# GestaltCogTeam/STEP

Measured on AMD Instinct MI355X. Metric: training windows/sec on PEMS04, horizon-12 MAE parity, 1/2/4/8 MI355X, higher is better.
Workload: dtype f16 (TSFormer Q/K/weights) + bf16 (P, V, GraphWaveNet / graph-learner GEMMs) operands, f32 accumulate

## Files before the change

include/step_hip.h:

```cpp
#ifndef STEP_HIP_H
#define STEP_HIP_H

#include <stdint.h>

#ifdef __cplusplus
extern "C" {
#endif

const char* step_last_error(void);
int step_abi_version(void);

typedef struct StepGemm {
    int M, N, K, batch;
    const void* A; long sam, sak, sab; int a_bf16;
    const void* B; long sbk, sbn, sbb; int b_bf16;
    float* C; long ldc, scn, scb;
    float alpha;
    int accumulate;
    const float* bias; int relu;
    int splitk;
    int a_kblk; long a_kstride;
    int b_kblk; long b_kstride;
    int b_nblk; long b_nstride;
    int c_nblk; long c_nstride;
// ... 42 lines not shown

long step_dgl_global_saved_floats(int N, int T);
long step_dgl_global_work_floats(int N, int T, int backward);
int step_dgl_global_forward(const float* series_nt, int N, int T, const StepDglParams* p, int training,
                            float momentum, float* saved, float* work, float* g, void* stream);
int step_dgl_global_backward(const float* series_nt, int N, int T, const StepDglParams* p, const float* saved,
                             const float* dg, float* work, const StepDglParams* grads, void* stream);
#define STEP_DGL_FRESH_FC_GRAD 16
int step_dgl_global_backward_phase(const float* series_nt, int N, int T, const StepDglParams* p, const float* saved,
                             const float* dg, float* work, const StepDglParams* grads, int phase, void* stream);

typedef struct StepDglShard { int own1; double count1, count2; } StepDglShard;
int step_dgl_global_forward_shard(const float* series_slice, int N, int Ts, const StepDglParams* p, int training, float momentum,
                                  float* saved, float* work, double* sums, float* g, const StepDglShard* shard, int phase,
                                  void* stream);
int step_dgl_global_backward_shard(const float* series_slice, int N, int Ts, const StepDglParams* p, const float* saved,
                                   const float* dg, float* work, const StepDglParams* grads, const StepDglShard* shard, int phase,
                                   void* stream);
long step_dgl_global_offset(int N, int T, int item);

int step_dgl_fc_dgrad(const float* dgpre, const void* wp, const void* a2h, const float* coef, const float* st2, int N, long K,
                      void* dz2h, void* stream);
long step_dgl_fc_dgrad_streams(int N, long K);

long step_dgl_edges_saved_floats(int B, int N);
long step_dgl_edges_work_floats(int N);
long step_dgl_edges_theta_offset(int N);
int step_dgl_edges_forward(const float* g, int N, int B, const StepDglParams* p, const float* u, uint64_t seed,
                           float temperature, float* saved, float* theta_out, float* adj_out, void* stream);
int step_dgl_edges_forward_keyed(const float* g, int N, int B, const StepDglParams* p, const long* key, uint64_t seed,
                                 float temperature, float* saved, float* theta_out, float* adj_out, void* stream);
int step_dgl_edges_backward(const float* g, int N, int B, const StepDglParams* p, const float* saved,
                            const float* dtheta, const float* dadj, float temperature, float* work,
                            const StepDglParams* grads, float* dg, void* aux_stream, void* stream);
int step_dgl_edges_backward_acc(const float* g, int N, int B, const StepDglParams* p, const float* saved,
                                const float* dtheta, const float* dadj, float temperature, float* work,
                                const StepDglParams* grads, float* dg, int dg_accumulate, void* aux_stream, void* stream);

typedef struct StepGwnetParams {
    float *nodevec1, *nodevec2;
    float *start_w, *start_b;
    float *filter_w[8], *filter_b[8];
    float *gate_w[8], *gate_b[8];
    float *skip_w[8], *skip_b[8];
    float *bn_w[8], *bn_b[8], *bn_rm[8], *bn_rv[8];
    float *gconv_w[8], *gconv_b[8];
// ... 171 lines not shown
```

step_amd/_lib.py:

```python
import ctypes
import os

import torch

_HERE = os.path.dirname(os.path.abspath(__file__))
LIB_PATH = os.environ.get("STEP_HIP_LIB") or os.path.join(_HERE, "libstep_hip.so")

_vp, _i, _l, _f, _u64 = ctypes.c_void_p, ctypes.c_int, ctypes.c_long, ctypes.c_float, ctypes.c_uint64


class StepGemm(ctypes.Structure):
    _fields_ = [("M", _i), ("N", _i), ("K", _i), ("batch", _i),
                ("A", _vp), ("sam", _l), ("sak", _l), ("sab", _l), ("a_bf16", _i),
                ("B", _vp), ("sbk", _l), ("sbn", _l), ("sbb", _l), ("b_bf16", _i),
                ("C", _vp), ("ldc", _l), ("scn", _l), ("scb", _l),
                ("alpha", _f), ("accumulate", _i), ("bias", _vp), ("relu", _i), ("splitk", _i),
                ("a_kblk", _i), ("a_kstride", _l), ("b_kblk", _i), ("b_kstride", _l),
                ("b_nblk", _i), ("b_nstride", _l), ("c_nblk", _i), ("c_nstride", _l),
                ("a_kscale", _vp), ("a_kshift", _vp), ("a_kperiod", _i),
                ("batch0", _i), ("sab1", _l), ("sbb1", _l), ("scb1", _l), ("compute_bf16", _i), ("a_rowsum", _vp), ("c_nscale", _vp), ("c_nshift", _vp), ("c_mvec", _vp),
                ("c_nperiod", _i), ("splitk_ws", _vp), ("splitk_ws_floats", _l)]


class StepDglParams(ctypes.Structure):
# ... 31 lines not shown
    "step_last_error": (ctypes.c_char_p, []),
    "step_abi_version": (_i, []),
    "step_gemm": (_i, [ctypes.POINTER(StepGemm), _vp]),
    "step_tsformer_encode": (_i, [_vp, _i, _i, _vp, _l, _i, _i, _vp, _vp, _vp, _vp, _f, _vp, _l, _u64, _vp, _vp]),
    "step_dropout_pool_fill": (_i, [_vp, _l, _f, _u64, _vp]),
    "step_tsformer_dropout_words": (_l, [_i, _i]),
    "step_gather_windows": (_i, [_vp, _i, _i, _i, _i, _vp, _i, _i, _i, _vp, _vp, _vp, _vp]),
    "step_pack_long_history": (_i, [_vp, _i, _i, _i, _i, _i, _vp, _vp]),
    "step_knn_workspace_bytes": (_l, [_i, _i, _i]),
    "step_knn_graph": (_i, [_vp, _vp, _i, _i, _i, _i, _vp, _vp, _vp, _l, _vp]),
    "step_topk_mask": (_i, [_vp, _i, _i, _i, _vp, _vp, _l, _vp]),
    "step_selftest_mfma": (_i, [_vp, _vp]),
    "step_streams_concurrent": (_i, [_vp, _vp, ctypes.POINTER(_i)]),
    "step_dgl_global_saved_floats": (_l, [_i, _i]),
    "step_dgl_global_work_floats": (_l, [_i, _i, _i]),
    "step_dgl_global_forward": (_i, [_vp, _i, _i, _PD, _i, _f, _vp, _vp, _vp, _vp]),
    "step_dgl_global_backward": (_i, [_vp, _i, _i, _PD, _vp, _vp, _vp, _PD, _vp]),
    "step_dgl_global_backward_phase": (_i, [_vp, _i, _i, _PD, _vp, _vp, _vp, _PD, _i, _vp]),
    "step_dgl_global_forward_shard": (_i, [_vp, _i, _i, _PD, _i, _f, _vp, _vp, _vp, _vp, _PS, _i, _vp]),
    "step_dgl_global_backward_shard": (_i, [_vp, _i, _i, _PD, _vp, _vp, _vp, _PD, _PS, _i, _vp]),
    "step_dgl_global_offset": (_l, [_i, _i, _i]),
    "step_dgl_fc_dgrad": (_i, [_vp, _vp, _vp, _vp, _vp, _i, _l, _vp, _vp]),
    "step_dgl_fc_dgrad_streams": (_l, [_i, _l]),
    "step_dgl_edges_saved_floats": (_l, [_i, _i]),
    "step_dgl_edges_work_floats": (_l, [_i]),
    "step_dgl_edges_theta_offset": (_l, [_i]),
    "step_dgl_edges_forward": (_i, [_vp, _i, _i, _PD, _vp, _u64, _f, _vp, _vp, _vp, _vp]),
    "step_dgl_edges_forward_keyed": (_i, [_vp, _i, _i, _PD, _vp, _u64, _f, _vp, _vp, _vp, _vp]),
    "step_dgl_edges_backward": (_i, [_vp, _i, _i, _PD, _vp, _vp, _vp, _f, _vp, _PD, _vp, _vp, _vp]),
    "step_dgl_edges_backward_acc": (_i, [_vp, _i, _i, _PD, _vp, _vp, _vp, _f, _vp, _PD, _vp, _i, _vp, _vp]),
    "step_gwnet_saved_floats": (_l, [_i, _i, _i]),
    "step_gwnet_work_floats": (_l, [_i, _i, _i]),
    "step_gwnet_saved_offset": (_l, [_i, _i, _i, _i, _i]),
    "step_gwnet_forward": (_i, [_vp, _i, _i, _i, _vp, _vp, _PG, _i, _f, _u64, _f, _vp, _vp, _vp, _vp]),
    "step_gwnet_forward_phase": (_i, [_vp, _i, _i, _i, _vp, _vp, _PG, _i, _f, _u64, _f, _vp, _vp, _vp, _i, _vp]),
    "step_gwnet_backward": (_i, [_vp, _i, _i, _i, _vp, _PG, _vp, _vp, _vp, _PG, _vp, _i, _vp, _vp, _vp]),
    "step_pt_dropout": (_i, [_vp, _vp, _l, _f, _u64, ctypes.c_uint32, _vp]),
    "step_pt_ffn_hidden_fwd": (_i, [_vp, _vp, _vp, _l, _f, _u64, ctypes.c_uint32, _vp, _vp]),
    "step_pt_ffn_hidden_bwd": (_i, [_vp, _vp, _vp, _l, _f, _vp, _vp]),
    "step_pt_colsum_bf16": (_i, [_vp, _l, _i, _vp, _vp]),
    "step_pt_rows_linear_pack_bytes": (_l, [_i, _i]),
    "step_pt_rows_linear_pack": (_i, [_vp, _l, _l, _i, _i, _vp, _vp, _vp]),
    "step_pt_rows_linear": (_i, [_vp, _i, _l, _vp, _i, _i, _vp, _i, _i, _vp]),
    "step_pt_layer_pack": (_i, [_vp] * 14),
    "step_pt_proj_wgrad_ws_floats": (_l, [_l]),
    "step_pt_proj_wgrad": (_i, [_vp, _vp, _vp, _vp, _l, _vp, _vp, _vp, _vp, _vp]),
# ... 152 lines not shown
```

step_amd/csrc/dgl.hip:

```cpp
#include "common.h"
#include "step_internal.h"

namespace {

constexpr int KW = 10;
constexpr int EMB = 100;

template <int CI, int CO, int TPT>
__global__ __launch_bounds__(256) void conv_relu_fwd_kernel(const float* __restrict__ in, const float* __restrict__ w,
                                                            const float* __restrict__ b, const float* __restrict__ in_sc,
                                                            const float* __restrict__ in_sh, float* __restrict__ out,
                                                            float* __restrict__ partial, int Tin, int stat_limit) {
    __shared__ __attribute__((aligned(16))) float ws[CI * KW * CO];
    __shared__ float red[4][2 * CO];
    const int tid = threadIdx.x, n = blockIdx.y;
    const int Tout = Tin - (KW - 1);
    for (int e = tid; e < CI * KW * CO; e += 256) {
        int co = e % CO, k = (e / CO) % KW, ci = e / (CO * KW);
        ws[e] = w[(co * CI + ci) * KW + k];
    }
    __syncthreads();
    const int t0 = (blockIdx.x * 256 + tid) * TPT;
    float acc[CO][TPT];
#pragma unroll
// ... 654 lines not shown
#pragma unroll
        for (int r = 0; r < 16; ++r) v += red[r][tid];
        atomicAdd(&dots_o[o * 32 + tid], v);
    }
}
__global__ void dots_reduce_kernel(const float* __restrict__ dots_o, float* __restrict__ dots) {
    const int i = threadIdx.x;
    if (i >= 32) return;
    double a = 0.0;
    for (int o = 0; o < EMB; ++o) a += dots_o[o * 32 + i];
    dots[i] = (float)a;
}

static bool dgl_channels_last(const StepDglParams* p) {
    const char* e = getenv("STEP_DGL_F32_STORAGE");
    return p->gemm_bf16 && !(e && e[0] == '1');
}

static bool dgl_fc_stream() {
    const char* e = getenv("STEP_DGL_FC_STREAM");
    return !(e && e[0] == '0' && e[1] == 0);
}

static int dgl_fc_dgrad(const float* dgpre, const void* wp, const void* a2h, const float* coef, const float* st2, int N, long K, void* dz2h,
                        hipStream_t st) {
    if (dgl_fc_stream() && dgl_fc_stream_dgrad_ok(N, K)) return dgl_fc_stream_dgrad(dgpre, wp, a2h, coef, st2, N, EMB, K, dz2h, st);
    StepGemm gm = gemm_desc(N, (int)K, EMB, dgpre, EMB, 1, (const float*)wp, K, 1, (float*)dz2h, K);
    gm.b_bf16 = 1;
    gm.compute_bf16 = 1;
    GemmFused fu = {nullptr, nullptr, (const float*)a2h, coef, st2, 16, (int)(K / 16), GEMM_FUSED_INTERLEAVED};
    return step_gemm_launch_fused(gm, fu, st);
}

extern "C" long step_dgl_fc_dgrad_streams(int N, long K) { return dgl_fc_stream() && dgl_fc_stream_dgrad_ok(N, K) ? 1 : 0; }

extern "C" int step_dgl_fc_dgrad(const float* dgpre, const void* wp, const void* a2h, const float* coef, const float* st2, int N, long K,
                                 void* dz2h, void* stream) {
    STEP_REQUIRE(dgpre && wp && a2h && coef && st2 && dz2h && N > 0 && K > 0 && K % 16 == 0 && K <= 0x7fffffffL, "dgl_fc_dgrad: bad arguments");
    STEP_REQUIRE(((((uintptr_t)dgpre) | ((uintptr_t)wp) | ((uintptr_t)a2h) | ((uintptr_t)dz2h)) & 15) == 0, "dgl_fc_dgrad: buffers must be 16-byte aligned");
    return dgl_fc_dgrad(dgpre, wp, a2h, coef, st2, N, K, dz2h, (hipStream_t)stream);
}

static bool dgl_legacy_bn_backward() {
    const char* e = getenv("STEP_DGL_LEGACY_BN");
    return e && e[0] == '1';
}

extern "C" long step_dgl_global_saved_floats(int N, int T) {
    long T1 = T - 9, T2 = T - 18;
    return (long)N * 8 * T1 + (long)N * 16 * T2 + (long)N * EMB + 4 * 8 + 4 * 16 + 4 * EMB + (long)EMB * 16 * T2 + 128;
}
static long fc_splitk_ws_floats(int N, int T2) {
    const int splits = step_gemm_auto_splitk(N, EMB, 16 * T2, 1);
    return splits > 1 ? (long)splits * N * EMB + 4 : 0;
}
static long wraw_floats(long T2) {
    const long w = (long)EMB * 16 * T2, pack = dgl_conv2_pack_floats();
    return w > pack ? w : pack;
}
extern "C" long step_dgl_global_work_floats(int N, int T, int backward) {
    long T1 = T - 9, T2 = T - 18;
    long nb1 = (long)N * cdiv(T1, 1024), nb2 = (long)N * cdiv(T2, 1024);
    long part = (nb1 > nb2 ? nb1 : nb2) * 32 + 64;
// ... 189 lines not shown
        float* colsum = coef + 128;
        if (do_fc) {
            bn3_relu_bwd_kernel<<<EMB, 256, 0, st>>>(dg, gpre, N, p->bn3_w, st3, grads->bn3_w, grads->bn3_b, grads->fc_b, dgpre, dgpreT, colsum);
            STEP_LAUNCH_CHECK("bn3_bwd");
            StepGemm gm = gemm_desc(EMB, (int)K, N, dgpre, 1, EMB, a2, K, 1, wraw, K);
            gm.b_bf16 = 1;
            gm.compute_bf16 = 1;
            if (dgl_fc_stream() && dgl_fc_stream_wgrad_ok(N)) STEP_TRY(dgl_fc_stream_wgrad(a2, dgpreT, N, EMB, K, wraw, st));
            else STEP_TRY(step_gemm_launch(gm, st));
            if (hipMemsetAsync(dots_o, 0, EMB * 32 * sizeof(float), st) != hipSuccess) { step_set_error("memset failed"); return STEP_ERR_HIP; }
            fc_unpermute_kernel<<<dim3(cdiv(T2, 256), EMB), 256, 0, st>>>(wraw, p->fc_w, st2, colsum, grads->fc_w, dots_o, T2, fresh_fc);
            dots_reduce_kernel<<<1, 64, 0, st>>>(dots_o, dots);
            STEP_LAUNCH_CHECK("fc_unpermute");
        }
        if (do_mid) {
            bn2_fused_coef_kernel<<<1, 64, 0, st>>>(dots, st2, p->bn2_w, count2, grads->bn2_w, grads->bn2_b, coef);
            STEP_LAUNCH_CHECK("bn2_fused_coef");
            STEP_TRY(dgl_fc_dgrad(dgpre, wp, a2, coef, st2, N, K, d_a2, st));
            STEP_TRY(dgl_conv2_wgrad_cl(d_a2, a1, wg_scratch, graw, N, T1, st));
        }
        if (do_tail) {
            STEP_TRY(dgl_conv2_wgrad_finish(graw, p->conv2_w, st1, p->bn1_w, p->bn1_b, count1, grads->conv2_w, grads->conv2_b, grads->bn1_w,
                                            grads->bn1_b, coef + 64, 1, st));
            STEP_TRY(dgl_conv2_dgrad_cl(d_a2, p->conv2_w, st1, d_a1, N, T1, a1, coef + 64, st1, shard ? shard->own1 : T1, wraw, st));
            STEP_TRY(dgl_conv1_wgrad_cl(d_a1, series_nt, wg_scratch, grads->conv1_w, grads->conv1_b, N, T, st));
        }
        return STEP_OK;
    }
    if (do_fc) {
        float* colsum = coef + 128;
        bn3_relu_bwd_kernel<<<EMB, 256, 0, st>>>(dg, gpre, N, p->bn3_w, st3, grads->bn3_w, grads->bn3_b, grads->fc_b, dgpre, dgpreT, colsum);
        STEP_LAUNCH_CHECK("bn3_bwd");
        {
            StepGemm gm = gemm_desc(EMB, (int)K, N, dgpre, 1, EMB, a2, K, 1, grads->fc_w, K);
            gm.accumulate = fresh_fc ? 0 : 1;
            gm.c_nscale = st2; gm.c_nshift = st2 + 16; gm.c_nperiod = T2; gm.c_mvec = colsum;
            gm.compute_bf16 = p->gemm_bf16;
            if (fuse2) {
                if (hipMemsetAsync(dots, 0, 32 * sizeof(float), st) != hipSuccess) { step_set_error("memset failed"); return STEP_ERR_HIP; }
                GemmFused fu = {p->fc_w, dots, nullptr, nullptr, nullptr, 16, T2};
                STEP_TRY(step_gemm_launch_fused(gm, fu, st));
            } else {
                STEP_TRY(step_gemm_launch(gm, st));
            }
        }
    }
    if (!do_mid && !do_tail) return STEP_OK;
    if (do_mid) {
// ... 173 lines not shown
```

step_amd/csrc/dgl_conv_mfma.hip:

```cpp
#include "common.h"
#include "step_internal.h"

namespace {

constexpr int KW = 10, CI = 8, CO = 16, C1_ = 8;
constexpr int FW_TT = 1024;

__device__ __forceinline__ uint32_t cvt2(float a, float b) {
    uint32_t r;
    asm("v_cvt_pk_bf16_f32 %0, %1, %2" : "=v"(r) : "v"(a), "v"(b));
    return r;
}
__device__ __forceinline__ bf16x8 as_frag(uint4 v) { return __builtin_bit_cast(bf16x8, v); }

__global__ __launch_bounds__(256) void conv2_fwd_mfma_kernel(const float* __restrict__ a1, const float* __restrict__ w,
                                                             const float* __restrict__ b, const float* __restrict__ sc,
                                                             const float* __restrict__ sh, float* __restrict__ a2,
                                                             float* __restrict__ partial, int T1) {
    __shared__ uint4 xs[FW_TT + 16];
    __shared__ float red[4][2 * CO];
    const int tid = threadIdx.x, lane = tid & 63, wave = tid >> 6, n = blockIdx.y;
    const int T2 = T1 - (KW - 1), t0 = blockIdx.x * FW_TT;
    const int ln = lane & 15, q = lane >> 4;

// ... 762 lines not shown
            if (ln >= KW) bv = make_uint4(0u, 0u, 0u, 0u);
            acc = __builtin_amdgcn_mfma_f32_16x16x32_bf16(as_frag(av), as_frag(bv), acc, 0, 0, 0);
        }
    }
    __syncthreads();
    if (wave > 0) {
#pragma unroll
        for (int e = 0; e < 4; ++e) red[wave - 1][lane][e] = acc[e];
    }
#pragma unroll
    for (int co = 0; co < C1; ++co) {
        const float sm = wave_sum_fast(bsum[co]);
        if (lane == 0) redb[wave][co] = sm;
    }
    __syncthreads();
    float* out = partial + ((long)blockIdx.y * gridDim.x + blockIdx.x) * W1_OUT;
    if (wave == 0 && q < 2 && ln < KW) {
#pragma unroll
        for (int e = 0; e < 4; ++e) out[(4 * q + e) * KW + ln] = acc[e] + red[0][lane][e] + red[1][lane][e] + red[2][lane][e];
    }
    if (tid < C1) out[C1 * KW + tid] = redb[0][tid] + redb[1][tid] + redb[2][tid] + redb[3][tid];
}


}

static int wgrad_slices(long nrows) {
    long s = nrows / 256;
    return (int)(s < 16 ? 16 : (s > 128 ? 128 : s));
}

int dgl_conv2_fwd_mfma(const float* a1, const float* w, const float* b, const float* sc, const float* sh, float* a2, float* partial,
                       int N, int T1, int* nblk, hipStream_t st) {
    const int T2 = T1 - (KW - 1);
    dim3 grid(cdiv(T2, FW_TT), N);
    conv2_fwd_mfma_kernel<<<grid, 256, 0, st>>>(a1, w, b, sc, sh, a2, partial, T1);
    STEP_LAUNCH_CHECK("conv2_fwd_mfma");
    *nblk = grid.x * grid.y;
    return STEP_OK;
}

int dgl_conv2_dgrad_mfma(const float* dz, const float* w, float* din, int N, int T1, const float* bnx, const float* coef, const float* stat,
                         int own, hipStream_t st) {
    conv2_dgrad_mfma_kernel<<<dim3(cdiv(T1, FW_TT), N), 256, 0, st>>>(dz, w, din, T1, bnx, coef, stat, own);
    STEP_LAUNCH_CHECK("conv2_dgrad_mfma");
    return STEP_OK;
// ... 50 lines not shown
    conv1_fwd_cl_kernel<<<grid, 256, 0, st>>>(x, w, b, (uint4*)a1h, partial, T, stat_limit);
    STEP_LAUNCH_CHECK("conv1_fwd_cl");
    *nblk = grid.x * grid.y;
    return STEP_OK;
}
long dgl_conv2_pack_floats() { return 8 * 64 * 4 + 16; }
int dgl_conv2_fwd_cl(const void* a1h, const float* w, const float* b, const float* sc, const float* sh, void* a2h, float* partial, int N,
                     int T1, int* nblk, float* pack, hipStream_t st) {
    const int T2 = T1 - (KW - 1);
    dim3 grid(cdiv(T2, FW_TT), N);
    conv2_pack_kernel<<<1, 512, 0, st>>>(w, b, sc, sh, (uint4*)pack);
    conv2_fwd_cl_kernel<<<grid, 256, 0, st>>>((const uint4*)a1h, (const uint4*)pack, (uint2*)a2h, partial, T1);
    STEP_LAUNCH_CHECK("conv2_fwd_cl");
    *nblk = grid.x * grid.y;
    return STEP_OK;
}
int dgl_conv2_dgrad_cl(const void* dz2h, const float* w, const float* sc, void* dz1h, int N, int T1, const void* a1h, const float* coef,
                       const float* stat, int own, float* pack, hipStream_t st) {
    conv2_pack_kernel<<<1, 512, 0, st>>>(w, w, sc, sc, (uint4*)pack);
    conv2_dgrad_cl_kernel<<<dim3(cdiv(T1, FW_TT), N), 256, 0, st>>>((const uint4*)dz2h, (const uint4*)pack, (uint2*)dz1h, T1, (const uint2*)a1h, coef, stat, own);
    STEP_LAUNCH_CHECK("conv2_dgrad_cl");
    return STEP_OK;
}
int dgl_conv2_wgrad_cl(const void* dz2h, const void* a1h, float* scratch, float* graw, int N, int T1, hipStream_t st) {
    const int T2 = T1 - (KW - 1);
    dim3 grid(cdiv(T2, WG_SC * WG_PASSES), N);
    if (hipMemsetAsync(graw, 0, WG_OUT * sizeof(float), st) != hipSuccess) { step_set_error("memset failed"); return STEP_ERR_HIP; }
    conv2_wgrad_cl_kernel<<<grid, 256, 0, st>>>((const uint4*)dz2h, (const uint4*)a1h, scratch, T1);
    STEP_LAUNCH_CHECK("conv2_wgrad_cl");
    conv_wgrad_reduce_kernel<<<dim3(cdiv(WG_OUT, 64), wgrad_slices(grid.x * grid.y)), 256, 0, st>>>(scratch, grid.x * grid.y, WG_OUT, CO * CI * KW, graw, graw + CO * CI * KW);
    STEP_LAUNCH_CHECK("conv2_wgrad_reduce");
    return STEP_OK;
}
int dgl_conv1_wgrad_cl(const void* dz1h, const float* x, float* scratch, float* dw, float* db, int N, int T, hipStream_t st) {
    const int T1 = T - (KW - 1);
    dim3 grid(cdiv(T1, WG_SC * WG_PASSES), N);
    conv1_wgrad_cl_kernel<<<grid, 256, 0, st>>>((const uint4*)dz1h, x, scratch, T);
    STEP_LAUNCH_CHECK("conv1_wgrad_cl");
    conv_wgrad_reduce_kernel<<<dim3(cdiv(W1_OUT, 64), wgrad_slices(grid.x * grid.y)), 256, 0, st>>>(scratch, grid.x * grid.y, W1_OUT, C1 * KW, dw, db);
    STEP_LAUNCH_CHECK("conv1_wgrad_reduce");
    return STEP_OK;
}
```

step_amd/csrc/dgl_fc_stream.hip:

```cpp
#include "common.h"
#include "step_internal.h"
#include "lds_dma.h"
#include <stdlib.h>

namespace {

template <int N>
__device__ __forceinline__ void fs_wait_vm() {
    static_assert(N >= 0 && N <= 63, "vmcnt");
    if constexpr (N == 0) asm volatile("s_waitcnt vmcnt(0)" ::: "memory");
    else if constexpr (N == 5) asm volatile("s_waitcnt vmcnt(5)" ::: "memory");
    else if constexpr (N == 6) asm volatile("s_waitcnt vmcnt(6)" ::: "memory");
    else if constexpr (N == 20) asm volatile("s_waitcnt vmcnt(20)" ::: "memory");
    else if constexpr (N == 40) asm volatile("s_waitcnt vmcnt(40)" ::: "memory");
    else if constexpr (N == 53) asm volatile("s_waitcnt vmcnt(53)" ::: "memory");
    else static_assert(N == 0, "add the case");
}
__device__ __forceinline__ void fs_barrier() {
    __builtin_amdgcn_s_barrier();
    asm volatile("" ::: "memory");
}

constexpr int FS_TM = 320, FS_KS = 64, FS_ROWB = FS_KS * 2, FS_WROWS = 104, FS_RING = 3, FS_WAVES = 10;
constexpr int FS_STAGE = (FS_TM + FS_WROWS) * FS_ROWB;
// ... 185 lines not shown
            acc0 = __builtin_amdgcn_mfma_f32_32x32x16_bf16(afr[2 * kb2], __builtin_bit_cast(bf16x8, b0), acc0, 0, 0, 0);
            acc1 = __builtin_amdgcn_mfma_f32_32x32x16_bf16(afr[2 * kb2 + 1], __builtin_bit_cast(bf16x8, b1), acc1, 0, 0, 0);
        }
        const long col = (long)(tile0 + i) * WG_CT + r;
        const int ob = wave * 32 + 4 * h;
        if (col < K) {
#pragma unroll
            for (int e = 0; e < 16; ++e) {
                const int o = ob + 8 * (e >> 2) + (e & 3);
                if (o < O) G[(long)o * K + col] = acc0[e] + acc1[e];
            }
        }
    }
}

constexpr int DG_TM = FS_TM, DG_CT = FS_KS, DG_ROWB = FS_ROWB, DG_WROWS = FS_WROWS, DG_RING = FS_RING, DG_STAGE = FS_STAGE;
constexpr int DG_MATH_WAVES = DG_TM / 64, DG_THREADS = (DG_MATH_WAVES + 1) * 64, DG_OMAX = 100, DG_KB = (DG_OMAX + 15) / 16;
constexpr int DG_LOADS = (DG_TM + DG_WROWS) / 8;
static_assert(DG_LOADS <= 63 && DG_WROWS % 8 == 0 && DG_WROWS >= 16 * (DG_KB - 1) + 8 && DG_RING * DG_STAGE <= 160 * 1024, "input-gradient stage");

__global__ __launch_bounds__(DG_THREADS) void fc_stream_dgrad_kernel(const float* __restrict__ D, const uint16_t* __restrict__ W,
                                                                     const uint16_t* __restrict__ A, const float* __restrict__ coef,
                                                                     const float* __restrict__ st2, int N, int O, long K, int per, int rtiles,
                                                                     uint16_t* __restrict__ out) {
    extern __shared__ __attribute__((aligned(16))) char fs_lds[];
    const int tid = threadIdx.x, lane = tid & 63, wave = __builtin_amdgcn_readfirstlane(tid >> 6);
    const int rt = blockIdx.x % rtiles, s = blockIdx.x / rtiles;
    const int row0 = rt * DG_TM;
    const int tiles = (int)((K + DG_CT - 1) / DG_CT);
    const int tile0 = s * per;
    const int ntile = min(tiles - tile0, per);
    if (ntile <= 0) return;
    if (wave == DG_MATH_WAVES) {
        const uint32_t lds0 = (uint32_t)(uintptr_t)(__attribute__((address_space(3))) char*)fs_lds;
        const int pca = (lane & 7) ^ (lane >> 3), pcw = (lane & 7) ^ (((lane >> 4) & 1) << 2);
        auto issue = [&](int tile, int buf) {
            const long c0 = (long)(tile0 + tile) * DG_CT;
            const long offa = c0 + (c0 + pca * 8 < K ? pca * 8 : 0), offw = c0 + (c0 + pcw * 8 < K ? pcw * 8 : 0);
            const uint32_t base = lds0 + (uint32_t)(buf * DG_STAGE);
#pragma unroll
            for (int j = 0; j < DG_TM / 8; ++j)
                lds_dma_1k(A + (long)min(row0 + j * 8 + (lane >> 3), N - 1) * K + offa, base + (uint32_t)(j * 1024));
#pragma unroll
            for (int j = 0; j < DG_WROWS / 8; ++j)
                lds_dma_1k(W + (long)min(j * 8 + (lane >> 3), O - 1) * K + offw, base + (uint32_t)(DG_TM * DG_ROWB + j * 1024));
        };
        issue(0, 0);
// ... 17 lines not shown
            for (int j = 0; j < 8; ++j) {
                const int o = kb * 16 + 8 * h + j;
                const float x = d[min(o, O - 1)];
                v[j] = o < O ? x : 0.f;
            }
            afr[t2][kb] = pack8(v);
        }
    }
    const int c = lane & 15;
    const float km1 = coef[32 + c] * coef[c], km2 = coef[32 + c] * coef[16 + c] * st2[48 + c], mu = st2[32 + c];
    const int q = (lane & 15) >> 2, qb = (q >> 1) & 1;
    int trw[2];
#pragma unroll
    for (int j = 0; j < 2; ++j) trw[j] = DG_TM * DG_ROWB + q * DG_ROWB + (j ^ qb) * 64 + ((lane >> 4) & 1) * 32 + (lane & 3) * 8;
    int xoff[4][2];
#pragma unroll
    for (int e3 = 0; e3 < 4; ++e3)
#pragma unroll
        for (int j = 0; j < 2; ++j) {
            const int r7 = e3 + 4 * h;
            xoff[e3][j] = (wave * 64 + r7) * DG_ROWB + (((j * 4 + (r >> 3)) ^ r7) << 4) + (r & 7) * 2;
        }
    const int pc = (lane & 7) ^ (lane >> 3);
    for (int i = 0; i < ntile; ++i) {
        fs_barrier();
        char* buf = fs_lds + (i % DG_RING) * DG_STAGE;
        f32x16 acc[4];
#pragma unroll
        for (int t = 0; t < 4; ++t)
#pragma unroll
            for (int e = 0; e < 16; ++e) acc[t][e] = 0.f;
#pragma unroll
        for (int kb = 0; kb < DG_KB; ++kb) {
            const int rowb = 16 * kb + 8 * h < DG_WROWS ? 16 * kb + 8 * h : 16 * kb;
            bf16x8 b[2];
#pragma unroll
            for (int j = 0; j < 2; ++j) {
                const char* p = buf + rowb * DG_ROWB + trw[j];
                const u32x2 lo = fs_read_tr(p), hi = fs_read_tr(p + 4 * DG_ROWB);
                const u32x4 t = {lo[0], lo[1], hi[0], hi[1]};
                b[j] = __builtin_bit_cast(bf16x8, t);
            }
            acc[0] = __builtin_amdgcn_mfma_f32_32x32x16_bf16(afr[0][kb], b[0], acc[0], 0, 0, 0);
            acc[1] = __builtin_amdgcn_mfma_f32_32x32x16_bf16(afr[0][kb], b[1], acc[1], 0, 0, 0);
            acc[2] = __builtin_amdgcn_mfma_f32_32x32x16_bf16(afr[1][kb], b[0], acc[2], 0, 0, 0);
            acc[3] = __builtin_amdgcn_mfma_f32_32x32x16_bf16(afr[1][kb], b[1], acc[3], 0, 0, 0);
        }
#pragma unroll
        for (int t = 0; t < 4; ++t) {
            uint16_t xb[16];
#pragma unroll
            for (int e = 0; e < 16; ++e) xb[e] = *(const uint16_t*)(buf + ((t >> 1) * 32 + 8 * (e >> 2)) * DG_ROWB + xoff[e & 3][t & 1]);
#pragma unroll
            for (int e = 0; e < 16; ++e) {
                const float x = __uint_as_float((uint32_t)xb[e] << 16);
                const float v = acc[t][e];
                const float o = x > 0.f ? v - km1 - (x - mu) * km2 : 0.f;
                *(uint16_t*)(buf + ((t >> 1) * 32 + 8 * (e >> 2)) * DG_ROWB + xoff[e & 3][t & 1]) = __builtin_bit_cast(uint16_t, (__bf16)o);
            }
        }
        asm volatile("s_waitcnt lgkmcnt(0)" ::: "memory");
        const long col = (long)(tile0 + i) * DG_CT + pc * 8;
        uint4 piece[8];
#pragma unroll
        for (int it = 0; it < 8; ++it) piece[it] = *(const uint4*)(buf + (wave * 64 + it * 8 + (lane >> 3)) * DG_ROWB + (lane & 7) * 16);
#pragma unroll
        for (int it = 0; it < 8; ++it) {
            const int row = row0 + wave * 64 + it * 8 + (lane >> 3);
            if (row < N && col < K) *(uint4*)(out + (long)row * K + col) = piece[it];
        }
    }
}

int env_int(const char* name, int dflt) {
    const char* e = getenv(name);
    return e && e[0] ? atoi(e) : dflt;
}

}

bool dgl_fc_stream_wgrad_ok(int N) { return N <= WG_TN; }

constexpr int FS_RANGES = 96;
int dgl_fc_stream_fwd(const void* a2h, const void* wp, int N, int O, long K, float* gpre, float* ws, long ws_floats, hipStream_t st) {
    STEP_REQUIRE(a2h && wp && gpre && N > 0 && O > 0 && O <= FS_WROWS && K > 0 && K % 16 == 0, "dgl_fc_stream_fwd: bad arguments");
    const int ksteps = (int)((K + FS_KS - 1) / FS_KS);
    const long mn = (long)N * O;
    long ranges = (ws && (((uintptr_t)ws) & 15) == 0) ? ws_floats / mn : 1;
    const int want = env_int("STEP_DGL_FC_STREAM_RANGES", FS_RANGES);
    if (ranges > want) ranges = want;
    if (ranges > ksteps) ranges = ksteps;
    if (ranges < 1) ranges = 1;
// ... 11 lines not shown
        STEP_LAUNCH_CHECK("dgl_fc_stream_fwd(reduce)");
    }
    return STEP_OK;
}

int dgl_fc_stream_wgrad(const void* a2h, const float* dgpreT, int N, int O, long K, float* G, hipStream_t st) {
    STEP_REQUIRE(a2h && dgpreT && G && N > 0 && N <= WG_TN && O > 0 && O <= WG_OROWS && K > 0 && K % 16 == 0, "dgl_fc_stream_wgrad: bad arguments");
    const int tiles = (int)((K + WG_CT - 1) / WG_CT);
    int groups = env_int("STEP_DGL_FC_STREAM_WGROUPS", 256);
    if (groups > tiles) groups = tiles;
    if (groups < 1) groups = 1;
    const int per = (tiles + groups - 1) / groups;
    STEP_TRY(step_raise_lds_once((const void*)fc_stream_wgrad_kernel, 160 * 1024, "dgl_fc_stream_wgrad"));
    fc_stream_wgrad_kernel<<<(tiles + per - 1) / per, WG_THREADS, WG_DBYTES + WG_RING * WG_STAGE, st>>>((const uint16_t*)a2h, dgpreT, N, O, K, per, G);
    STEP_LAUNCH_CHECK("dgl_fc_stream_wgrad");
    return STEP_OK;
}

constexpr int DG_MAX_RTILES = 3;
bool dgl_fc_stream_dgrad_ok(int N, long K) { return N > 0 && N <= DG_MAX_RTILES * DG_TM && K > 0; }

constexpr int DG_GROUPS = 256;
int dgl_fc_stream_dgrad(const float* dgpre, const void* wp, const void* a2h, const float* coef, const float* st2, int N, int O, long K,
                        void* dz2h, hipStream_t st) {
    STEP_REQUIRE(dgpre && wp && a2h && coef && st2 && dz2h && N > 0 && O > 0 && O <= DG_OMAX && K > 0 && K % 16 == 0,
                 "dgl_fc_stream_dgrad: bad arguments");
    STEP_REQUIRE(((((uintptr_t)wp) | ((uintptr_t)a2h) | ((uintptr_t)dz2h)) & 15) == 0, "dgl_fc_stream_dgrad: wp, a2h and dz2h must be 16-byte aligned");
    const int tiles = (int)((K + DG_CT - 1) / DG_CT), rtiles = cdiv(N, DG_TM);
    int ranges = env_int("STEP_DGL_FC_STREAM_DGROUPS", DG_GROUPS) / rtiles;
    if (ranges > tiles) ranges = tiles;
    if (ranges < 1) ranges = 1;
    const int per = (tiles + ranges - 1) / ranges;
    const int used = (tiles + per - 1) / per;
    STEP_TRY(step_raise_lds_once((const void*)fc_stream_dgrad_kernel, 160 * 1024, "dgl_fc_stream_dgrad"));
    fc_stream_dgrad_kernel<<<used * rtiles, DG_THREADS, DG_RING * DG_STAGE, st>>>(dgpre, (const uint16_t*)wp, (const uint16_t*)a2h, coef, st2, N, O, K, per,
                                                                                 rtiles, (uint16_t*)dz2h);
    STEP_LAUNCH_CHECK("dgl_fc_stream_dgrad");
    return STEP_OK;
}
```

step_amd/csrc/step_internal.h:

```cpp
#pragma once
#include <hip/hip_runtime.h>
#include <vector>
#include "../../include/step_hip.h"

enum { GEMM_FUSED_INTERLEAVED = 1, GEMM_FUSED_FFN_FWD = 2, GEMM_FUSED_MASKNZ = 4, GEMM_FUSED_BF16OUT = 8 };
struct GemmFused {
    const float* dotw; float* dots;
    const float* bnx; const float* bncoef; const float* bnstat;
    int channels, period;
    int flags;
    const float* ffn_bias; const void* maskx; float p; unsigned seed_lo, seed_hi, site;
};

struct GemmKSeg { long a_off, b_off, a_bs, b_bs; int a_rs, b_rs; };
constexpr int GEMM_KSEG_MAX = 128;
int step_gemm_segmented_launch(StepGemm g, const GemmKSeg* ktab, int ktab_per, hipStream_t st);

int step_gemm_launch(StepGemm g, hipStream_t st);
int step_gemm_auto_splitk(int M, int N, int K, int batch);
int step_gemm_launch_fused(StepGemm g, const GemmFused& fused, hipStream_t st);
int step_gemm_bf16_launch(StepGemm g, hipStream_t st, const GemmFused* fused = nullptr);
int step_gemm_f32_fast_launch(StepGemm g, hipStream_t st, const GemmFused* fused = nullptr);

static inline StepGemm gemm_desc(int M, int N, int K, const float* A, long sam, long sak, const float* B, long sbk,
// ... 5 lines not shown
    g.B = B; g.sbk = sbk; g.sbn = sbn;
    g.C = C; g.ldc = ldc; g.scn = 1;
    g.alpha = 1.f; g.splitk = 1;
    return g;
}

int step_gemm_rowsum_separate(StepGemm* g, hipStream_t st);
int dgl_conv2_fwd_mfma(const float* a1, const float* w, const float* b, const float* sc, const float* sh, float* a2, float* partial,
                       int N, int T1, int* nblk, hipStream_t st);
int dgl_conv2_dgrad_mfma(const float* dz, const float* w, float* din, int N, int T1, const float* bnx, const float* coef, const float* stat,
                         int own, hipStream_t st);
int dgl_conv2_wgrad_xhat_mfma(const float* dz, const float* a1, const float* stat1, float* scratch, float* graw, int N, int T1, hipStream_t st);
int dgl_conv2_wgrad_finish(const float* graw, const float* w, const float* stat1, const float* gamma1, const float* beta1, double count,
                           float* dw, float* db, float* dgamma1, float* dbeta1, float* coef1, int raw, hipStream_t st);
int dgl_conv1_fwd_cl(const float* x, const float* w, const float* b, void* a1h, float* partial, int N, int T, int stat_limit, int* nblk,
                     hipStream_t st);
long dgl_conv2_pack_floats();
int dgl_conv2_fwd_cl(const void* a1h, const float* w, const float* b, const float* sc, const float* sh, void* a2h, float* partial, int N,
                     int T1, int* nblk, float* pack, hipStream_t st);
int dgl_conv2_dgrad_cl(const void* dz2h, const float* w, const float* sc, void* dz1h, int N, int T1, const void* a1h, const float* coef,
                       const float* stat, int own, float* pack, hipStream_t st);
int dgl_conv2_wgrad_cl(const void* dz2h, const void* a1h, float* scratch, float* graw, int N, int T1, hipStream_t st);
int dgl_conv1_wgrad_cl(const void* dz1h, const float* x, float* scratch, float* dw, float* db, int N, int T, hipStream_t st);
long dgl_conv2_wgrad_scratch_floats(int N, int T1);
int dgl_conv2_wgrad_mfma(const float* dz, const float* a1, const float* sc, const float* sh, float* scratch, float* dw, float* db, int N,
                         int T1, hipStream_t st);
int dgl_conv1_wgrad_mfma(const float* dz, const float* x, float* scratch, float* dw, float* db, int N, int T, hipStream_t st);
int dgl_fc_stream_fwd(const void* a2h, const void* wp, int N, int O, long K, float* gpre, float* ws, long ws_floats, hipStream_t st);
bool dgl_fc_stream_wgrad_ok(int N);
int dgl_fc_stream_wgrad(const void* a2h, const float* dgpreT, int N, int O, long K, float* G, hipStream_t st);
bool dgl_fc_stream_dgrad_ok(int N, long K);
int dgl_fc_stream_dgrad(const float* dgpre, const void* wp, const void* a2h, const float* coef, const float* st2, int N, int O, long K,
                        void* dz2h, hipStream_t st);
int step_colsum_launch(const float* x, long rows, int cols, long ld, float* out, hipStream_t st);

struct AuxLane {
    hipStream_t main, aux;
    bool on;
    int next = 0, base = 0;
    AuxLane(hipStream_t m, hipStream_t a, int base_ = 0) : main(m), aux(a), on(a != nullptr && a != m), base(base_) {}
    static hipEvent_t event(int k) {
        thread_local std::vector<hipEvent_t> pool[16];
        int dev = 0;
        (void)hipGetDevice(&dev);
        std::vector<hipEvent_t>& v = pool[dev & 15];
        while ((int)v.size() <= k) {
            hipEvent_t e;
            if (hipEventCreateWithFlags(&e, hipEventDisableTiming) != hipSuccess) return nullptr;
            v.push_back(e);
        }
        return v[k];
    }
    hipStream_t fork() {
        if (!on) return main;
        hipEvent_t e = event(base + (next++ & 63));
        if (!e || hipEventRecord(e, main) != hipSuccess || hipStreamWaitEvent(aux, e, 0) != hipSuccess) { on = false; return main; }
// ... 36 lines not shown
```

Measured before the change: 2479.

## Fuse conv2 data-gradient with conv1 weight-gradient and add pitched fc dgrad output

Adds a kernel that computes the conv2 data-gradient tile and immediately uses it, staged in shared memory, to form conv1 weight-gradient partials. This avoids writing dz1 to global memory and reading it back in a separate kernel. The fused path is on by default and can be disabled with an environment variable. The fc streaming dgrad kernel also gains a row pitch and a store-alignment carry scheme that delays each store by one tile when rows are misaligned, and a pitched entry point is exposed; this adds register pressure and extra logic.

```diff
diff --git a/include/step_hip.h b/include/step_hip.h
--- a/include/step_hip.h
+++ b/include/step_hip.h
@@ -88,6 +88,8 @@
 int step_dgl_fc_dgrad(const float* dgpre, const void* wp, const void* a2h, const float* coef, const float* st2, int N, long K,
                       void* dz2h, void* stream);
 long step_dgl_fc_dgrad_streams(int N, long K);
+int step_dgl_fc_dgrad_pitched(const float* dgpre, const void* wp, const void* a2h, const float* coef, const float* st2, int N, long K,
+                              void* dz2h, long pitch, void* stream);
 
 long step_dgl_edges_saved_floats(int B, int N);
 long step_dgl_edges_work_floats(int N);
diff --git a/step_amd/_lib.py b/step_amd/_lib.py
--- a/step_amd/_lib.py
+++ b/step_amd/_lib.py
@@ -77,6 +77,7 @@
     "step_dgl_global_offset": (_l, [_i, _i, _i]),
     "step_dgl_fc_dgrad": (_i, [_vp, _vp, _vp, _vp, _vp, _i, _l, _vp, _vp]),
     "step_dgl_fc_dgrad_streams": (_l, [_i, _l]),
+    "step_dgl_fc_dgrad_pitched": (_i, [_vp, _vp, _vp, _vp, _vp, _i, _l, _vp, _l, _vp]),
     "step_dgl_edges_saved_floats": (_l, [_i, _i]),
     "step_dgl_edges_work_floats": (_l, [_i]),
     "step_dgl_edges_theta_offset": (_l, [_i]),
diff --git a/step_amd/csrc/dgl.hip b/step_amd/csrc/dgl.hip
--- a/step_amd/csrc/dgl.hip
+++ b/step_amd/csrc/dgl.hip
@@ -700,9 +700,14 @@
     return !(e && e[0] == '0' && e[1] == 0);
 }
 
+static bool dgl_dz1_fused() {
+    const char* e = getenv("STEP_DGL_DZ1_FUSED");
+    return !(e && e[0] == '0' && e[1] == 0);
+}
+
 static int dgl_fc_dgrad(const float* dgpre, const void* wp, const void* a2h, const float* coef, const float* st2, int N, long K, void* dz2h,
                         hipStream_t st) {
-    if (dgl_fc_stream() && dgl_fc_stream_dgrad_ok(N, K)) return dgl_fc_stream_dgrad(dgpre, wp, a2h, coef, st2, N, EMB, K, dz2h, st);
+    if (dgl_fc_stream() && dgl_fc_stream_dgrad_ok(N, K)) return dgl_fc_stream_dgrad(dgpre, wp, a2h, coef, st2, N, EMB, K, dz2h, K, st);
     StepGemm gm = gemm_desc(N, (int)K, EMB, dgpre, EMB, 1, (const float*)wp, K, 1, (float*)dz2h, K);
     gm.b_bf16 = 1;
     gm.compute_bf16 = 1;
@@ -717,6 +722,15 @@
     STEP_REQUIRE(dgpre && wp && a2h && coef && st2 && dz2h && N > 0 && K > 0 && K % 16 == 0 && K <= 0x7fffffffL, "dgl_fc_dgrad: bad arguments");
     STEP_REQUIRE(((((uintptr_t)dgpre) | ((uintptr_t)wp) | ((uintptr_t)a2h) | ((uintptr_t)dz2h)) & 15) == 0, "dgl_fc_dgrad: buffers must be 16-byte aligned");
     return dgl_fc_dgrad(dgpre, wp, a2h, coef, st2, N, K, dz2h, (hipStream_t)stream);
+}
+
+extern "C" int step_dgl_fc_dgrad_pitched(const float* dgpre, const void* wp, const void* a2h, const float* coef, const float* st2, int N, long K,
+                                         void* dz2h, long pitch, void* stream) {
+    STEP_REQUIRE(dgpre && wp && a2h && coef && st2 && dz2h && N > 0 && K > 0 && K % 16 == 0 && K <= 0x7fffffffL && pitch >= K && pitch % 8 == 0,
+                 "dgl_fc_dgrad_pitched: bad arguments");
+    STEP_REQUIRE(((((uintptr_t)dgpre) | ((uintptr_t)wp) | ((uintptr_t)a2h) | ((uintptr_t)dz2h)) & 15) == 0, "dgl_fc_dgrad_pitched: buffers must be 16-byte aligned");
+    STEP_REQUIRE(dgl_fc_stream_dgrad_ok(N, K), "dgl_fc_dgrad_pitched: the size is outside the streaming kernel's");
+    return dgl_fc_stream_dgrad(dgpre, wp, a2h, coef, st2, N, EMB, K, dz2h, pitch, (hipStream_t)stream);
 }
 
 static bool dgl_legacy_bn_backward() {
@@ -952,8 +966,13 @@
         if (do_tail) {
             STEP_TRY(dgl_conv2_wgrad_finish(graw, p->conv2_w, st1, p->bn1_w, p->bn1_b, count1, grads->conv2_w, grads->conv2_b, grads->bn1_w,
                                             grads->bn1_b, coef + 64, 1, st));
-            STEP_TRY(dgl_conv2_dgrad_cl(d_a2, p->conv2_w, st1, d_a1, N, T1, a1, coef + 64, st1, shard ? shard->own1 : T1, wraw, st));
-            STEP_TRY(dgl_conv1_wgrad_cl(d_a1, series_nt, wg_scratch, grads->conv1_w, grads->conv1_b, N, T, st));
+            if (dgl_dz1_fused()) {
+                STEP_TRY(dgl_conv2_dgrad_c1w_cl(d_a2, p->conv2_w, st1, N, T1, a1, coef + 64, st1, shard ? shard->own1 : T1, wraw, series_nt, wg_scratch, grads->conv1_w,
+                                                grads->conv1_b, st));
+            } else {
+                STEP_TRY(dgl_conv2_dgrad_cl(d_a2, p->conv2_w, st1, d_a1, N, T1, a1, coef + 64, st1, shard ? shard->own1 : T1, wraw, st));
+                STEP_TRY(dgl_conv1_wgrad_cl(d_a1, series_nt, wg_scratch, grads->conv1_w, grads->conv1_b, N, T, st));
+            }
         }
         return STEP_OK;
     }
diff --git a/step_amd/csrc/dgl_conv_mfma.hip b/step_amd/csrc/dgl_conv_mfma.hip
--- a/step_amd/csrc/dgl_conv_mfma.hip
+++ b/step_amd/csrc/dgl_conv_mfma.hip
@@ -808,6 +808,145 @@
     if (tid < C1) out[C1 * KW + tid] = redb[0][tid] + redb[1][tid] + redb[2][tid] + redb[3][tid];
 }
 
+__global__ __launch_bounds__(256) void conv2_dgrad_c1w_cl_kernel(const uint4* __restrict__ dz2h, const uint4* __restrict__ pack, int T1,
+                                                                 const uint2* __restrict__ a1h, const float* __restrict__ coef,
+                                                                 const float* __restrict__ stat, int own, const float* __restrict__ x,
+                                                                 float* __restrict__ partial) {
+    constexpr int ZP = FW_TT + 8, XP = FW_TT + 16;
+    constexpr int Z1_BYTES = C1 * ZP * 2, X_BYTES = XP * 2, RED_BYTES = 3 * 64 * 4 * 4, REDB_BYTES = 4 * C1 * 4;
+    __shared__ uint4 zs[FW_TT + 16][2];
+    static_assert(Z1_BYTES % 16 == 0 && X_BYTES % 16 == 0 && Z1_BYTES + 2 * X_BYTES + RED_BYTES + REDB_BYTES <= (int)sizeof(zs),
+                  "the weight-gradient images live in the dz2 window");
+    const int tid = threadIdx.x, lane = tid & 63, wave = tid >> 6, n = blockIdx.y;
+    const int T2 = T1 - (KW - 1), T = T1 + (KW - 1), t0 = blockIdx.x * FW_TT;
+    const int ln = lane & 15, q = lane >> 4;
+    constexpr int NT = FW_TT / 16 / 4;
+    uint2 xall[NT];
+    if (q < 2) {
+#pragma unroll
+        for (int i = 0; i < NT; ++i) {
+            const int t = t0 + (wave + 4 * i) * 16 + ln;
+            xall[i] = t < T1 ? a1h[((long)n * T1 + t) * 2 + q] : make_uint2(0u, 0u);
+        }
+    }
+    constexpr int NLD = (FW_TT + 16 + 255) / 256;
+    float xs[NLD];
+#pragma unroll
+    for (int u = 0; u < NLD; ++u) xs[u] = x[(long)n * T + min(t0 + tid + 256 * u, T - 1)];
+    {
+        uint4 r0[NLD], r1[NLD];
+#pragma unroll
+        for (int u = 0; u < NLD; ++u) {
+            const int t = max(min(t0 - (KW - 1) + min(tid + 256 * u, FW_TT + 15), T2 - 1), 0);
+            r0[u] = dz2h[((long)n * T2 + t) * 2];
+            r1[u] = dz2h[((long)n * T2 + t) * 2 + 1];
+        }
+#pragma unroll
+        for (int u = 0; u < NLD; ++u) {
+            const int tt = tid + 256 * u, t = t0 - (KW - 1) + tt;
+            const bool ok = t >= 0 && t < T2;
+            if (tt < FW_TT + 16) {
+                zs[tt][0] = ok ? r0[u] : make_uint4(0u, 0u, 0u, 0u);
+                zs[tt][1] = ok ? r1[u] : make_uint4(0u, 0u, 0u, 0u);
+            }
+        }
+    }
+    bf16x8 wf[5];
+#pragma unroll
+    for (int s = 0; s < 5; ++s) wf[s] = as_frag(pack[(3 + s) * 64 + lane]);
+    float km1[4] = {0.f, 0.f, 0.f, 0.f}, km2[4] = {0.f, 0.f, 0.f, 0.f}, mu[4] = {0.f, 0.f, 0.f, 0.f};
+    if (q < 2) {
+#pragma unroll
+        for (int e = 0; e < 4; ++e) {
+            const int c = 4 * q + e;
+            km1[e] = coef[2 * CI + c] * coef[c]; km2[e] = coef[2 * CI + c] * coef[CI + c] * stat[3 * CI + c]; mu[e] = stat[2 * CI + c];
+        }
+    }
+    __syncthreads();
+    float bs[4] = {0.f, 0.f, 0.f, 0.f};
+#pragma unroll
+    for (int i = 0; i < NT; ++i) {
+        const int tb = (wave + 4 * i) * 16;
+        uint2 ov = make_uint2(0u, 0u);
+        if (t0 + tb < T1) {
+            f32x4 acc = {0.f, 0.f, 0.f, 0.f};
+#pragma unroll
+            for (int s = 0; s < 5; ++s) {
+                const int kk = 2 * s + (q >> 1);
+                acc = __builtin_amdgcn_mfma_f32_16x16x32_bf16(wf[s], as_frag(zs[tb + ln + (KW - 1) - kk][q & 1]), acc, 0, 0, 0);
+            }
+            const int t = t0 + tb + ln;
+            if (t < T1 && q < 2) {
+                const float xv[4] = {bf16lo(xall[i].x), bf16hi(xall[i].x), bf16lo(xall[i].y), bf16hi(xall[i].y)};
+                float o[4];
+#pragma unroll
+                for (int e = 0; e < 4; ++e) o[e] = xv[e] > 0.f ? acc[e] - (t < own ? km1[e] + (xv[e] - mu[e]) * km2[e] : 0.f) : 0.f;
+                ov = make_uint2(cvt2(o[0], o[1]), cvt2(o[2], o[3]));
+                bs[0] += bf16lo(ov.x); bs[1] += bf16hi(ov.x); bs[2] += bf16lo(ov.y); bs[3] += bf16hi(ov.y);
+            }
+        }
+        xall[i] = ov;
+    }
+    __syncthreads();
+    char* base = (char*)&zs[0][0];
+    uint16_t (*z1)[ZP] = (uint16_t (*)[ZP])base;
+    uint16_t* x0 = (uint16_t*)(base + Z1_BYTES);
+    uint16_t* x1 = (uint16_t*)(base + Z1_BYTES + X_BYTES);
+    float (*red)[64][4] = (float (*)[64][4])(base + Z1_BYTES + 2 * X_BYTES);
+    float (*redb)[C1] = (float (*)[C1])(base + Z1_BYTES + 2 * X_BYTES + RED_BYTES);
+    if (q < 2) {
+#pragma unroll
+        for (int i = 0; i < NT; ++i) {
+            const int tt = (wave + 4 * i) * 16 + ln;
+            z1[4 * q][tt] = (uint16_t)(xall[i].x & 0xffffu); z1[4 * q + 1][tt] = (uint16_t)(xall[i].x >> 16);
+            z1[4 * q + 2][tt] = (uint16_t)(xall[i].y & 0xffffu); z1[4 * q + 3][tt] = (uint16_t)(xall[i].y >> 16);
+        }
+    }
+#pragma unroll
+    for (int u = 0; u < NLD; ++u) {
+        const int tt = tid + 256 * u;
+        if (tt < XP) {
+            const uint16_t hv = (uint16_t)(cvt2(t0 + tt < T ? xs[u] : 0.f, 0.f) & 0xffffu);
+            x0[tt] = hv;
+            if (tt > 0) x1[tt - 1] = hv;
+        }
+    }
+    if (tid == 0) x1[XP - 1] = 0;
+#pragma unroll
+    for (int e = 0; e < 4; ++e) {
+        const float sm = row_sum_fast(bs[e]);
+        if (ln == 15 && q < 2) redb[wave][4 * q + e] = sm;
+    }
+    __syncthreads();
+    f32x4 acc = {0.f, 0.f, 0.f, 0.f};
+#pragma unroll
+    for (int g = 0; g < FW_TT / 256 * 2; ++g) {
+        const int tg = (g >> 1) * 256 + 64 * wave + 32 * (g & 1);
+        if (t0 + tg < T1) {
+            const int tb = tg + 8 * q;
+            uint4 av = *(const uint4*)&z1[ln & 7][tb];
+            if (ln >= C1) av = make_uint4(0u, 0u, 0u, 0u);
+            const int kk = ln < KW ? ln : 0;
+            const uint16_t* row = (kk & 1) ? x1 : x0;
+            const uint32_t* p = (const uint32_t*)(row + tb + (kk & ~1));
+            uint4 bv = make_uint4(p[0], p[1], p[2], p[3]);
+            if (ln >= KW) bv = make_uint4(0u, 0u, 0u, 0u);
+            acc = __builtin_amdgcn_mfma_f32_16x16x32_bf16(as_frag(av), as_frag(bv), acc, 0, 0, 0);
+        }
+    }
+    if (wave > 0) {
+#pragma unroll
+        for (int e = 0; e < 4; ++e) red[wave - 1][lane][e] = acc[e];
+    }
+    __syncthreads();
+    float* out = partial + ((long)blockIdx.y * gridDim.x + blockIdx.x) * W1_OUT;
+    if (wave == 0 && q < 2 && ln < KW) {
+#pragma unroll
+        for (int e = 0; e < 4; ++e) out[(4 * q + e) * KW + ln] = acc[e] + red[0][lane][e] + red[1][lane][e] + red[2][lane][e];
+    }
+    if (tid < C1) out[C1 * KW + tid] = redb[0][tid] + redb[1][tid] + redb[2][tid] + redb[3][tid];
+}
+
 
 }
 
@@ -904,6 +1043,19 @@
     STEP_LAUNCH_CHECK("conv2_dgrad_cl");
     return STEP_OK;
 }
+int dgl_conv2_dgrad_c1w_cl(const void* dz2h, const float* w, const float* sc, int N, int T1, const void* a1h, const float* coef,
+                           const float* stat, int own, float* pack, const float* x, float* scratch, float* dw, float* db, hipStream_t st) {
+    dim3 grid(cdiv(T1, FW_TT), N);
+    STEP_REQUIRE((long)grid.x * grid.y * W1_OUT <= dgl_conv2_wgrad_scratch_floats(N, T1), "dgl_conv2_dgrad_c1w_cl: partial rows exceed the scratch buffer");
+    conv2_pack_kernel<<<1, 512, 0, st>>>(w, w, sc, sc, (uint4*)pack);
+    conv2_dgrad_c1w_cl_kernel<<<grid, 256, 0, st>>>((const uint4*)dz2h, (const uint4*)pack, T1, (const uint2*)a1h, coef, stat, own, x, scratch);
+    STEP_LAUNCH_CHECK("conv2_dgrad_c1w_cl");
+    const long nrows = (long)grid.x * grid.y;
+    const int slices = (int)(nrows / 32 < 16 ? 16 : (nrows / 32 > 256 ? 256 : nrows / 32));
+    conv_wgrad_reduce_kernel<<<dim3(cdiv(W1_OUT, 64), slices), 256, 0, st>>>(scratch, grid.x * grid.y, W1_OUT, C1 * KW, dw, db);
+    STEP_LAUNCH_CHECK("conv1_wgrad_reduce");
+    return STEP_OK;
+}
 int dgl_conv2_wgrad_cl(const void* dz2h, const void* a1h, float* scratch, float* graw, int N, int T1, hipStream_t st) {
     const int T2 = T1 - (KW - 1);
     dim3 grid(cdiv(T2, WG_SC * WG_PASSES), N);
diff --git a/step_amd/csrc/dgl_fc_stream.hip b/step_amd/csrc/dgl_fc_stream.hip
--- a/step_amd/csrc/dgl_fc_stream.hip
+++ b/step_amd/csrc/dgl_fc_stream.hip
@@ -231,7 +231,7 @@
 __global__ __launch_bounds__(DG_THREADS) void fc_stream_dgrad_kernel(const float* __restrict__ D, const uint16_t* __restrict__ W,
                                                                      const uint16_t* __restrict__ A, const float* __restrict__ coef,
                                                                      const float* __restrict__ st2, int N, int O, long K, int per, int rtiles,
-                                                                     uint16_t* __restrict__ out) {
+                                                                     uint16_t* __restrict__ out, long ldo) {
     extern __shared__ __attribute__((aligned(16))) char fs_lds[];
     const int tid = threadIdx.x, lane = tid & 63, wave = __builtin_amdgcn_readfirstlane(tid >> 6);
     const int rt = blockIdx.x % rtiles, s = blockIdx.x / rtiles;
@@ -295,6 +295,10 @@
             xoff[e3][j] = (wave * 64 + r7) * DG_ROWB + (((j * 4 + (r >> 3)) ^ r7) << 4) + (r & 7) * 2;
         }
     const int pc = (lane & 7) ^ (lane >> 3);
+    const bool trail = (int)((((uintptr_t)(out + (long)(row0 + wave * 64 + (lane >> 3)) * ldo)) >> 4) & 7) + pc >= 8;
+    uint4 carry[8];
+#pragma unroll
+    for (int it = 0; it < 8; ++it) carry[it] = make_uint4(0u, 0u, 0u, 0u);
     for (int i = 0; i < ntile; ++i) {
         fs_barrier();
         char* buf = fs_lds + (i % DG_RING) * DG_STAGE;
@@ -337,10 +341,22 @@
         uint4 piece[8];
 #pragma unroll
         for (int it = 0; it < 8; ++it) piece[it] = *(const uint4*)(buf + (wave * 64 + it * 8 + (lane >> 3)) * DG_ROWB + (lane & 7) * 16);
+        const long scol = trail ? col - DG_CT : col;
+        const bool live = !trail || i > 0;
 #pragma unroll
         for (int it = 0; it < 8; ++it) {
             const int row = row0 + wave * 64 + it * 8 + (lane >> 3);
-            if (row < N && col < K) *(uint4*)(out + (long)row * K + col) = piece[it];
+            const uint4 v = trail ? carry[it] : piece[it];
+            if (live && row < N && scol < K) *(uint4*)(out + (long)row * ldo + scol) = v;
+            carry[it] = piece[it];
+        }
+    }
+    if (trail) {
+        const long col = (long)(tile0 + ntile - 1) * DG_CT + pc * 8;
+#pragma unroll
+        for (int it = 0; it < 8; ++it) {
+            const int row = row0 + wave * 64 + it * 8 + (lane >> 3);
+            if (row < N && col < K) *(uint4*)(out + (long)row * ldo + col) = carry[it];
         }
     }
 }
@@ -398,8 +414,8 @@
 
 constexpr int DG_GROUPS = 256;
 int dgl_fc_stream_dgrad(const float* dgpre, const void* wp, const void* a2h, const float* coef, const float* st2, int N, int O, long K,
-                        void* dz2h, hipStream_t st) {
-    STEP_REQUIRE(dgpre && wp && a2h && coef && st2 && dz2h && N > 0 && O > 0 && O <= DG_OMAX && K > 0 && K % 16 == 0,
+                        void* dz2h, long pitch, hipStream_t st) {
+    STEP_REQUIRE(dgpre && wp && a2h && coef && st2 && dz2h && N > 0 && O > 0 && O <= DG_OMAX && K > 0 && K % 16 == 0 && pitch >= K && pitch % 8 == 0,
                  "dgl_fc_stream_dgrad: bad arguments");
     STEP_REQUIRE(((((uintptr_t)wp) | ((uintptr_t)a2h) | ((uintptr_t)dz2h)) & 15) == 0, "dgl_fc_stream_dgrad: wp, a2h and dz2h must be 16-byte aligned");
     const int tiles = (int)((K + DG_CT - 1) / DG_CT), rtiles = cdiv(N, DG_TM);
@@ -410,7 +426,7 @@
     const int used = (tiles + per - 1) / per;
     STEP_TRY(step_raise_lds_once((const void*)fc_stream_dgrad_kernel, 160 * 1024, "dgl_fc_stream_dgrad"));
     fc_stream_dgrad_kernel<<<used * rtiles, DG_THREADS, DG_RING * DG_STAGE, st>>>(dgpre, (const uint16_t*)wp, (const uint16_t*)a2h, coef, st2, N, O, K, per,
-                                                                                 rtiles, (uint16_t*)dz2h);
+                                                                                 rtiles, (uint16_t*)dz2h, pitch);
     STEP_LAUNCH_CHECK("dgl_fc_stream_dgrad");
     return STEP_OK;
 }
diff --git a/step_amd/csrc/step_internal.h b/step_amd/csrc/step_internal.h
--- a/step_amd/csrc/step_internal.h
+++ b/step_amd/csrc/step_internal.h
@@ -51,6 +51,8 @@
                        const float* stat, int own, float* pack, hipStream_t st);
 int dgl_conv2_wgrad_cl(const void* dz2h, const void* a1h, float* scratch, float* graw, int N, int T1, hipStream_t st);
 int dgl_conv1_wgrad_cl(const void* dz1h, const float* x, float* scratch, float* dw, float* db, int N, int T, hipStream_t st);
+int dgl_conv2_dgrad_c1w_cl(const void* dz2h, const float* w, const float* sc, int N, int T1, const void* a1h, const float* coef,
+                           const float* stat, int own, float* pack, const float* x, float* scratch, float* dw, float* db, hipStream_t st);
 long dgl_conv2_wgrad_scratch_floats(int N, int T1);
 int dgl_conv2_wgrad_mfma(const float* dz, const float* a1, const float* sc, const float* sh, float* scratch, float* dw, float* db, int N,
                          int T1, hipStream_t st);
@@ -60,7 +62,7 @@
 int dgl_fc_stream_wgrad(const void* a2h, const float* dgpreT, int N, int O, long K, float* G, hipStream_t st);
 bool dgl_fc_stream_dgrad_ok(int N, long K);
 int dgl_fc_stream_dgrad(const float* dgpre, const void* wp, const void* a2h, const float* coef, const float* st2, int N, int O, long K,
-                        void* dz2h, hipStream_t st);
+                        void* dz2h, long pitch, hipStream_t st);
 int step_colsum_launch(const float* x, long rows, int cols, long ld, float* out, hipStream_t st);
 
 struct AuxLane {
```

Result: no change. 2492, median of 3 (+0.5%).
